# granne/granne

Measured on AMD Instinct MI355X. Metric: queries/sec (recall@10 alongside), 10M x 100-d angular, batch=1024, higher is better.
Workload: dtype f32; 1 GPU; C2 (BASELINE.json configs[1]): 10000000 x 100-d f32 angular, i.i.d. uniform components, batch=1024, ef_search=50, k=10; n_elements=10000000, dim=100, batch=1024, ef_search=50, k=10

## Files before the change

### granne_amd/_lib.py

```python
import ctypes as C
import os

from . import build as _build

F32, I8 = 0, 1
UNUSED = 0xFFFFFFFF
BUILD_ALL = 0xFFFFFFFFFFFFFFFF

OK = 0
ERR_INVALID, ERR_HIP, ERR_NO_DEVICE, ERR_OVERFLOW, ERR_IO = -1, -2, -3, -4, -5

OPT_VISITED_SLOTS, OPT_FORCE_SLOW, OPT_SLOW_SLOTS, OPT_SLOW_BLOCKS, OPT_OVERFLOW_SLOTS = 1, 2, 3, 4, 5
OPT_VISITED16, OPT_VISITED16_LG, OPT_LAST_WALKER, OPT_SEARCH_DEPTH, OPT_INLINE_TAILS, OPT_SEEN_MIN = 6, 7, 8, 9, 10, 11
OPT_SKETCH = 12
OPT_COALESCE, OPT_COALESCE_MAX, OPT_COALESCE_WAIT_US, OPT_COALESCED_LAUNCHES, OPT_COALESCED_QUERIES = 13, 14, 15, 16, 17
COALESCE_CALL_MAX = 64
COALESCE_MAX = 1024
WALKER_NONE, WALKER_REGISTER, WALKER_REGISTER_WIDE, WALKER_GENERAL, WALKER_EXACT = 0, 1, 2, 3, 4
SEARCH_DEPTH = 3
SEARCH_DEPTH_MAX = 16
SHARDED_OPT_DEPTH, SHARDED_OPT_EXCHANGE = 1, 2
SHARDED_EXCHANGE_PEER, SHARDED_EXCHANGE_RCCL = 0, 1
RW_OPT_SMALL_OPS, RW_OPT_SMALL_LAUNCHES, RW_OPT_SORTED_LAUNCHES = 1, 2, 3
RW_SMALL_OPS = 2048
SE_MATERIALIZED, SE_COMPACT = 0, 1


class GranneHipError(RuntimeError):
    def __init__(self, code, message):
        super().__init__("granne_hip error %d: %s" % (code, message))
        self.code = code


class BuildConfig(C.Structure):
    _fields_ = [
        ("layer_multiplier", C.c_float),
        ("expected_num_elements", C.c_uint64),
        ("num_neighbors", C.c_uint32),
# ... 170 lines not shown
```

### granne_amd/csrc/granne_hip.hip

```cpp
#include <hip/hip_runtime.h>

#include <atomic>
#include <chrono>
#include <cstdarg>
#include <cstdio>
#include <cstdlib>
#include <cstring>
#include <memory>
#include <mutex>
#include <string>
#include <type_traits>
#include <vector>

#include "../../include/granne_hip.h"
#include "search_kernel.h"
#include "walk_fast.h"
#include "slow_kernel.h"
#include "util_kernels.h"
#include "brute_force.h"
#include "combiner.h"

using namespace granne_hip;

static_assert(Combiner::DEPTH <= GRANNE_HIP_SEARCH_DEPTH && Combiner::CALL_MAX == GRANNE_HIP_COALESCE_CALL_MAX &&
// ... 28 lines not shown
        if (hipGetDevice(&prev) != hipSuccess) prev = -1;
        ok = hipSetDevice(dev) == hipSuccess;
    }
    ~DeviceGuard() {
        if (prev >= 0) (void)hipSetDevice(prev);
    }
};

extern "C" const char* granne_hip_last_error(void) { return g_last_error.c_str(); }
extern "C" int granne_hip_abi_version(void) { return GRANNE_HIP_ABI_VERSION; }
extern "C" int granne_hip_device_count(int* out_count) {
    if (!out_count) return fail(GRANNE_HIP_ERR_INVALID, "out_count is null");
    int n = 0;
    hipError_t e = hipGetDeviceCount(&n);
    if (e != hipSuccess) {
        *out_count = 0;
        return fail(GRANNE_HIP_ERR_NO_DEVICE, "hipGetDeviceCount: %s", hipGetErrorString(e));
    }
    *out_count = n;
    return GRANNE_HIP_OK;
}

struct EnvKnobs {
    int visited = 0, touch_max = -1, inline_tails = 1, seen_min = -1, bf_b16 = 1, bf_ring = 1, sketch = 1;
    EnvKnobs() {
        auto geti = [](const char* name, int dflt) {
            const char* e = getenv(name);
            return e ? atoi(e) : dflt;
        };
        visited = geti("GRANNE_HIP_VISITED", 0);
        inline_tails = geti("GRANNE_HIP_INLINE_TAILS", 1);
        bf_ring = geti("GRANNE_HIP_BF_RING", 1);
        bf_b16 = geti("GRANNE_HIP_BF_B16", 1);
        seen_min = geti("GRANNE_HIP_SEEN_MIN", -1);
        touch_max = geti("GRANNE_HIP_TOUCH_MAX", -1);
        sketch = geti("GRANNE_HIP_SKETCH", 1);
    }
};
static const EnvKnobs& knobs() {
    static const EnvKnobs k;
    return k;
}

struct ScratchCache {
    struct Block {
        hipStream_t stream;
        uint8_t* p;
        size_t cap;
        uint64_t last_use;
        uint32_t small_runs;
        std::chrono::steady_clock::time_point last_time;
    };
    std::mutex mu;
    std::vector<Block> blocks;
    uint64_t uses = 0;
    std::vector<uint8_t*> graveyard;
    void free_all() {
        for (auto& b : blocks)
            if (b.p) (void)hipFree(b.p);
        blocks.clear();
        for (auto* p : graveyard) (void)hipFree(p);
        graveyard.clear();
    }
};

struct SeDev {
    int device = 0;
    uint32_t dim = 0, tstride = 0;
    uint64_t n_embeddings = 0, n = 0, n_terms = 0;
    float* d_table = nullptr;
    uint64_t* d_offsets = nullptr;
    uint32_t* d_terms = nullptr;
    uint64_t bytes() const { return n_embeddings * tstride * 4u + (n + 1) * 8u + n_terms * 4u; }
    ~SeDev() {
        DeviceGuard g(device);
        if (d_table) (void)hipFree(d_table);
        if (d_offsets) (void)hipFree(d_offsets);
        if (d_terms) (void)hipFree(d_terms);
    }
// ... 16 lines not shown
struct granne_hip_index {
    int device = 0;
    uint32_t dim = 0;
    int dtype = 0;
    uint64_t n_elements = 0;
    uint32_t row_bytes = 0;
    uint32_t row_stride = 0;
    uint8_t* d_elements = nullptr;
    std::shared_ptr<SeDev> se;
    std::vector<LayerHost> layers;
    LayerDev* d_layers = nullptr;
    uint64_t hbm_bytes = 0;
    uint32_t max_dev_width = 32;
    uint64_t opt_visited_slots = 0;
    uint64_t opt_force_slow = 0;
    uint64_t opt_slow_slots = 1u << 18;
    uint64_t opt_slow_blocks = 16;
    uint64_t opt_overflow_slots = 0;
    uint64_t opt_visited16 = 0;
    uint64_t opt_visited16_lg = 0;
    uint64_t opt_inline_tails = 1;
    uint64_t opt_seen_min = 2048;
    uint64_t opt_sketch = 1;
    std::atomic<uint64_t> last_slow_count{0};
    std::atomic<uint64_t> last_walker{0};
    std::mutex norm_mu;
    float* d_inv_norm = nullptr;
    uint8_t* d_sketch = nullptr;
    struct HostCall {
        hipStream_t stream = nullptr;
        uint8_t* d_buf = nullptr;
        size_t d_cap = 0;
        uint8_t* h_pin = nullptr;
        size_t h_cap = 0;
    };
    std::mutex call_mu;
    std::vector<HostCall*> call_free;
    uint64_t opt_coalesce = 0;
    Combiner combiner;
    HostCall* group_call[Combiner::DEPTH] = {};
    ScratchCache scratch;
    struct Flight {
        hipStream_t stream = nullptr;
        hipEvent_t ready = nullptr, done = nullptr;
        bool busy = false;
        uint64_t seq = 0;
// ... 497 lines not shown
        if (value < 1 || value > GRANNE_HIP_SEARCH_DEPTH_MAX) return fail(GRANNE_HIP_ERR_INVALID, "search depth must be in [1, %d]", GRANNE_HIP_SEARCH_DEPTH_MAX);
        std::lock_guard<std::mutex> lk(ix->flight_mu);
        for (auto& f : ix->flights)
            if (f.busy) return fail(GRANNE_HIP_ERR_INVALID, "the depth cannot change while a batch is in flight");
        ix->depth = (uint32_t)value;
        ix->next_flight = 0;
        return GRANNE_HIP_OK;
    }
    case GRANNE_HIP_OPT_INLINE_TAILS: {
        if (value > 1) return fail(GRANNE_HIP_ERR_INVALID, "the inline-tails option is 0 or 1");
        DeviceGuard g(ix->device);
        if (!g.ok) return fail(GRANNE_HIP_ERR_NO_DEVICE, "cannot select HIP device %d", ix->device);
        HIP_TRY(hipDeviceSynchronize());
        ix->opt_inline_tails = value;
        return finish_layers(ix, nullptr);
    }
    case GRANNE_HIP_OPT_SEEN_MIN:
        ix->opt_seen_min = value > 0xFFFFFFFFull ? 0xFFFFFFFFull : value;
        return GRANNE_HIP_OK;
    case GRANNE_HIP_OPT_SKETCH:
        if (value > 1) return fail(GRANNE_HIP_ERR_INVALID, "the sketch option is 0 or 1");
        ix->opt_sketch = value;
        return GRANNE_HIP_OK;
    case GRANNE_HIP_OPT_VISITED16_LG:
        if (value > 12) return fail(GRANNE_HIP_ERR_INVALID, "value out of range");
        ix->opt_visited16_lg = value;
        return GRANNE_HIP_OK;
    case GRANNE_HIP_OPT_COALESCE:
        if (value > 1) return fail(GRANNE_HIP_ERR_INVALID, "the coalesce option is 0 or 1");
        ix->opt_coalesce = value;
        return GRANNE_HIP_OK;
    case GRANNE_HIP_OPT_COALESCE_MAX:
        if (value < 1 || value > GRANNE_HIP_COALESCE_MAX) return fail(GRANNE_HIP_ERR_INVALID, "the coalesce cap must be in [1, %d]", GRANNE_HIP_COALESCE_MAX);
        ix->combiner.set_cap((uint32_t)value);
        return GRANNE_HIP_OK;
    case GRANNE_HIP_OPT_COALESCE_WAIT_US:
        ix->combiner.set_wait_us(value);
        return GRANNE_HIP_OK;
    case GRANNE_HIP_OPT_COALESCED_LAUNCHES:
    case GRANNE_HIP_OPT_COALESCED_QUERIES:
        return fail(GRANNE_HIP_ERR_INVALID, "option %d is read-only", option);
    default:
        return fail(GRANNE_HIP_ERR_INVALID, "unknown option %d", option);
    }
}

extern "C" int granne_hip_index_get_option(const granne_hip_index* ix, int option, uint64_t* value) {
    if (!ix || !value) return fail(GRANNE_HIP_ERR_INVALID, "null argument");
    switch (option) {
    case GRANNE_HIP_OPT_VISITED_SLOTS: *value = ix->opt_visited_slots; return GRANNE_HIP_OK;
    case GRANNE_HIP_OPT_FORCE_SLOW: *value = ix->opt_force_slow; return GRANNE_HIP_OK;
    case GRANNE_HIP_OPT_SLOW_SLOTS: *value = ix->opt_slow_slots; return GRANNE_HIP_OK;
    case GRANNE_HIP_OPT_SLOW_BLOCKS: *value = ix->opt_slow_blocks; return GRANNE_HIP_OK;
    case GRANNE_HIP_OPT_OVERFLOW_SLOTS: *value = ix->opt_overflow_slots; return GRANNE_HIP_OK;
    case GRANNE_HIP_OPT_VISITED16: *value = ix->opt_visited16; return GRANNE_HIP_OK;
    case GRANNE_HIP_OPT_VISITED16_LG: *value = ix->opt_visited16_lg; return GRANNE_HIP_OK;
    case GRANNE_HIP_OPT_LAST_WALKER: *value = ix->last_walker.load(); return GRANNE_HIP_OK;
    case GRANNE_HIP_OPT_SEARCH_DEPTH: *value = ix->depth; return GRANNE_HIP_OK;
    case GRANNE_HIP_OPT_INLINE_TAILS: *value = (!ix->layers.empty() && ix->layers.back().d_adjx) ? 1 : 0; return GRANNE_HIP_OK;
    case GRANNE_HIP_OPT_SEEN_MIN: *value = ix->opt_seen_min; return GRANNE_HIP_OK;
    case GRANNE_HIP_OPT_SKETCH: *value = (ix->opt_sketch && ix->d_sketch && knobs().sketch) ? 1 : 0; return GRANNE_HIP_OK;
    case GRANNE_HIP_OPT_COALESCE: *value = ix->opt_coalesce; return GRANNE_HIP_OK;
    case GRANNE_HIP_OPT_COALESCE_MAX: *value = ix->combiner.cap(); return GRANNE_HIP_OK;
    case GRANNE_HIP_OPT_COALESCE_WAIT_US: *value = ix->combiner.wait_us(); return GRANNE_HIP_OK;
    case GRANNE_HIP_OPT_COALESCED_LAUNCHES: *value = ix->combiner.launches(); return GRANNE_HIP_OK;
    case GRANNE_HIP_OPT_COALESCED_QUERIES: *value = ix->combiner.queries(); return GRANNE_HIP_OK;
    default: return fail(GRANNE_HIP_ERR_INVALID, "unknown option %d", option);
    }
}

extern "C" uint64_t granne_hip_index_last_slow_count(const granne_hip_index* ix) {
    return ix ? ix->last_slow_count.load() : 0;
}

constexpr size_t SLOW_SCRATCH_BUDGET = (size_t)1 << 30;
constexpr uint32_t SCRATCH_MAX_REGIONS = 16384;
constexpr size_t SCRATCH_STATE_OFF = CTL_WORDS * 4;
constexpr size_t SCRATCH_FIXED = SCRATCH_STATE_OFF + (size_t)SCRATCH_MAX_REGIONS * 4;

constexpr size_t SCRATCH_CACHE_STREAMS = 64;
constexpr int SCRATCH_IDLE_SECONDS = 10;
constexpr size_t SCRATCH_SHRINK_ABOVE = 256u << 20;

static int scratch_for(ScratchCache* cache, hipStream_t s, size_t total, uint8_t** out, bool* transient) {
    *transient = false;
    ScratchCache::Block* b = nullptr;
    cache->uses += 1;
    for (auto& x : cache->blocks)
        if (x.stream == s) b = &x;
// ... 35 lines not shown
        HIP_TRY(hipMalloc((void**)&b->p, want));
        b->cap = want;
        HIP_TRY(hipMemsetAsync(b->p, 0, SCRATCH_FIXED, s));
    }
    *out = b->p;
    return GRANNE_HIP_OK;
}

namespace {
struct SearchTarget {
    int device;
    const uint8_t* d_elements;
    uint64_t n_elements;
    uint32_t dim;
    int dtype;
    uint32_t row_bytes, row_stride;
    const LayerDev* d_layers;
    uint32_t n_layers;
    uint32_t max_dev_width;
    uint64_t opt_visited_slots = 0, opt_force_slow = 0, opt_slow_slots = 1u << 18, opt_slow_blocks = 16, opt_overflow_slots = 0;
    uint64_t opt_visited16 = 0;
    uint64_t opt_seen_min = 0xFFFFFFFFull;
    const uint8_t* d_sketch = nullptr;
    const SeDev* se = nullptr;
    ScratchCache* scratch;
    std::atomic<uint64_t>* last_walker = nullptr;

    template <class G>
    SearchTarget(const G* g, const LayerDev* layers, uint32_t n_layers)
        : device(g->device), d_elements(g->d_elements), n_elements(g->n_elements), dim(g->dim), dtype(g->dtype),
          row_bytes(g->row_bytes), row_stride(g->row_stride), d_layers(layers), n_layers(n_layers),
          scratch(&const_cast<G*>(g)->scratch) {
        if constexpr (std::is_same<G, granne_hip_index>::value) {
            max_dev_width = g->max_dev_width;
            opt_visited_slots = g->opt_visited_slots;
            opt_force_slow = g->opt_force_slow;
            opt_slow_slots = g->opt_slow_slots;
            opt_slow_blocks = g->opt_slow_blocks;
            opt_overflow_slots = g->opt_overflow_slots;
            opt_visited16 = g->opt_visited16;
            opt_seen_min = g->opt_seen_min;
            d_sketch = (g->opt_sketch && knobs().sketch) ? g->d_sketch : nullptr;
            last_walker = &const_cast<G*>(g)->last_walker;
            se = g->se.get();
        } else {
            max_dev_width = g->W;
        }
    }
};
}

struct SearchCall {
    const void* queries = nullptr;
    int64_t q_stride = 0;
    uint32_t nq = 0, ef = 0, k = 0;
    uint64_t* ids = nullptr;
    float* dists = nullptr;
    uint32_t* counts = nullptr;
    uint64_t* stats = nullptr;
    uint32_t* status = nullptr;
    hipStream_t stream = nullptr;
    uint32_t* slow_count = nullptr;
    uint32_t* trail = nullptr;
    uint32_t trail_layers = 0;
    hipEvent_t ev_before = nullptr, ev_after = nullptr;
// ... 262 lines not shown
    size_t total = off_sex + (T.se ? (size_t)W.slow_blocks * 64u * T.dim * 4u : 0u);
    struct Bury {
        std::vector<uint8_t*> blocks;
        ~Bury() {
            for (auto* b : blocks) (void)hipFree(b);
        }
    } bury;
    std::unique_lock<std::mutex> cache_lock(T.scratch->mu);
    uint8_t* scratch = nullptr;
    bool transient = false;
    {
        int r = scratch_for(T.scratch, s, total, &scratch, &transient);
        bury.blocks.swap(T.scratch->graveyard);
        if (r) return r;
    }
    struct FreeTransient {
        uint8_t* p;
        hipStream_t s;
        ~FreeTransient() {
            if (p) (void)hipFreeAsync(p, s);
        }
    } free_transient{transient ? scratch : nullptr, s};
    uint32_t* ctl = (uint32_t*)scratch;

    SlowParams sp;
    SearchParams& p = sp.sp;
    p.elements = T.d_elements;
    p.n_elements = T.n_elements;
    p.dim = T.dim;
    p.row_bytes = T.row_bytes;
    p.row_stride = T.row_stride;
    p.layers = T.d_layers;
    p.n_layers = T.n_layers;
    p.queries = (const uint8_t*)c.queries;
    p.q_stride = c.q_stride ? c.q_stride : (int64_t)T.dim * elem_size(T.dtype);
    p.nq = nq;
    p.ef = c.ef;
    p.k = c.k;
    p.out_ids = c.ids;
    p.out_dists = c.dists;
    p.out_counts = c.counts;
    p.out_stats = c.stats;
    p.visited_slots = W.visited_slots;
    p.upper_slots = W.upper_slots;
    p.front_eighths = W.front_eighths;
    p.maxc = W.maxc;
    p.lrow_bytes = W.lrow_bytes;
    p.stage_bytes = W.stage_bytes;
    p.adjspec_bytes = W.adjspec_bytes;
    p.slow_count = ctl + CTL_SLOW_COUNT;
    p.slow_list = (uint32_t*)(scratch + off_list);
    p.force_slow = 0;
    p.spec = 1;
    p.sketch = T.d_sketch;
    p.ovf.tables = (uint32_t*)(scratch + off_ovf);
    p.ovf.state = (uint32_t*)(scratch + SCRATCH_STATE_OFF);
    p.ovf.slots = W.ovf_slots;
    p.ovf.stride = W.ovf_slots;
    p.ovf.regions = W.ovf_regions;
    p.ovf.spilled = c.status ? c.status + 2 : ctl + CTL_SPILLED;
    p.trail_out = c.trail;
    p.trail_layers = c.trail_layers;
    p.n_batches = c.n_batches;
    p.batch_nq = batch_nq;
    for (uint32_t b = 0; b < c.n_batches; ++b) p.batch[b] = c.batches[b];
    sp.ctl = ctl;
    sp.vis = (uint32_t*)(scratch + off_vis);
    sp.pq = (uint64_t*)(scratch + off_pq);
    sp.res = (uint64_t*)(scratch + off_res);
    sp.slots = slots;
    sp.all = W.walker == GRANNE_HIP_WALKER_EXACT ? 1u : 0u;
    sp.status2 = c.status;
    sp.host_status = c.host_status;
    p.se_table = T.se ? T.se->d_table : nullptr;
    p.se_offsets = T.se ? T.se->d_offsets : nullptr;
    p.se_terms = T.se ? T.se->d_terms : nullptr;
    sp.se_x = T.se ? (float*)(scratch + off_sex) : nullptr;
// ... 919 lines not shown
```

### granne_amd/csrc/search_kernel.h

```cpp
#pragma once

#include "dist.h"
#include "wave_prims.h"
#include "sum_embeddings.h"

namespace granne_hip {

constexpr int DT_F32 = 0;
constexpr int DT_I8 = 1;

struct LayerDev {
    const uint32_t* adj;
    uint64_t len;
    uint32_t width;
    uint32_t flags;
    const uint8_t* adjx;
    uint32_t adjx_stride;
    uint32_t reserved;
};
constexpr uint32_t LAYER_TWIN_ROWS = 1u;

constexpr uint32_t SKETCH_LINE = 128u;
constexpr uint32_t SKETCH_META = 112u;
constexpr uint32_t SKETCH_MAX_DIM = 112u;
// ... 17 lines not shown
    const LayerDev* layers;
    uint32_t n_layers;
    const uint8_t* queries;
    int64_t q_stride;
    uint32_t nq;
    uint32_t ef;
    uint32_t k;
    uint64_t* out_ids;
    float* out_dists;
    uint32_t* out_counts;
    uint64_t* out_stats;
    uint32_t visited_slots;
    uint32_t upper_slots;
    uint32_t front_eighths;
    uint32_t maxc;
    uint32_t lrow_bytes;
    uint32_t stage_bytes;
    uint32_t adjspec_bytes;
    uint32_t* slow_count;
    uint32_t* slow_list;
    uint32_t force_slow;
    uint32_t spec;
    const uint8_t* sketch;
    OverflowPool ovf;
    uint32_t* trail_out;
    uint32_t trail_layers;
    uint32_t n_batches;
    uint32_t batch_nq;
    BatchIO batch[MAX_LAUNCH_BATCHES];
    const float* se_table;
    const uint64_t* se_offsets;
    const uint32_t* se_terms;
};
constexpr uint32_t TRAIL_WIDTH = 8;

struct QueryIO {
    const uint8_t* q;
    uint64_t* ids;
    float* dists;
    uint32_t* count;
    uint64_t* stats;
};
__device__ __forceinline__ QueryIO query_io(const SearchParams& p, uint32_t qi) {
    const uint8_t* q = p.queries;
    uint64_t* ids = p.out_ids;
    float* dists = p.out_dists;
// ... 467 lines not shown
```

### granne_amd/csrc/slow_kernel.h

```cpp
#pragma once

#include "search_kernel.h"

namespace granne_hip {

constexpr uint32_t CTL_SLOW_COUNT = 0;
constexpr uint32_t CTL_DONE = 1;
constexpr uint32_t CTL_TAIL_DONE = 2;
constexpr uint32_t CTL_EXHAUSTED = 3;
constexpr uint32_t CTL_LAST_SLOW = 4;
constexpr uint32_t CTL_LAST_EXHAUSTED = 5;
constexpr uint32_t CTL_SPILLED = 6;
constexpr uint32_t CTL_WORDS = 16;

struct SlowParams {
    SearchParams sp;
    uint32_t* ctl;
    uint32_t* vis;
    uint64_t* pq;
    uint64_t* res;
    uint32_t slots;
    uint32_t all;
    uint32_t* status2;
    uint32_t* host_status;
    float* se_x;
};

__device__ inline void gheap_push_min(uint64_t* h, uint32_t& n, uint64_t k) {
    uint32_t i = n++;
    while (i > 0) {
        uint32_t pa = (i - 1) >> 1;
        if (h[pa] <= k) break;
        h[i] = h[pa];
        i = pa;
    }
// ... 252 lines not shown
                uint64_t key = ok ? res[e] : KEY_INF;
                io.ids[e] = ok ? (uint64_t)key_id(key) : ~0ull;
                io.dists[e] = ok ? key_dist(key) : __builtin_inff();
            }
            *io.count = count;
            if (io.stats) {
                io.stats[0] = n_dist;
                io.stats[1] = n_expand;
                io.stats[2] = n_adj;
            }
        }
        __syncthreads();
    }
}

__device__ inline void slow_epilogue(const SlowParams& P, const uint32_t n_blocks, const uint32_t n_slow) {
    __syncthreads();
    if (threadIdx.x == 0) {
        __threadfence();
        if (atomicAdd(P.ctl + CTL_TAIL_DONE, 1u) == n_blocks - 1u) {
            const uint32_t ex = atomicExch(P.ctl + CTL_EXHAUSTED, 0u);
            atomicExch(P.ctl + CTL_LAST_SLOW, n_slow);
            atomicExch(P.ctl + CTL_LAST_EXHAUSTED, ex);
            atomicExch(P.ctl + CTL_SLOW_COUNT, 0u);
            atomicExch(P.ctl + CTL_DONE, 0u);
            atomicExch(P.ctl + CTL_TAIL_DONE, 0u);
        }
    }
}

__device__ __forceinline__ void walker_done(const SlowParams& P) {
    if (threadIdx.x == 0) atomicAdd(P.ctl + CTL_DONE, 1u);
}

template <int DT, bool SE = false>
__device__ inline void tail_block(const SlowParams& P, uint8_t* smem) {
    const uint32_t nq = P.sp.nq;
    const uint32_t me = blockIdx.x - nq, n_blocks = gridDim.x - nq;
    if (threadIdx.x == 0) {
        while (__hip_atomic_load(P.ctl + CTL_DONE, __ATOMIC_RELAXED, __HIP_MEMORY_SCOPE_AGENT) < nq)
            __builtin_amdgcn_s_sleep(24);
    }
    __syncthreads();
    const uint32_t n_slow = __hip_atomic_load(P.ctl + CTL_SLOW_COUNT, __ATOMIC_RELAXED, __HIP_MEMORY_SCOPE_AGENT);
    if (n_slow) slow_walk_list<DT, SE>(P, me, n_blocks, n_slow, smem);
    else if (me == 0 && threadIdx.x == 0 && P.host_status) P.host_status[1] = 0u;
// ... 23 lines not shown
```

### granne_amd/csrc/walk_fast.h

```cpp
#pragma once

#include <type_traits>

#include "slow_kernel.h"

namespace granne_hip {

#ifndef GRANNE_HIP_PHASE_TIMERS
#define GRANNE_HIP_PHASE_TIMERS 0
#endif
#if GRANNE_HIP_PHASE_TIMERS
constexpr uint32_t PHASE_SLOTS = 48, PHASE_QUERIES = 4096;
__device__ uint64_t g_phase[PHASE_QUERIES * PHASE_SLOTS];
#define PT_MARK(i)                                                                   \
    do {                                                                             \
        asm volatile("" ::: "memory");                                               \
        __builtin_amdgcn_sched_barrier(0);                                           \
        const uint64_t now_ = __builtin_amdgcn_s_memtime();                          \
        const uint64_t dt_ = now_ - pt_last;                                         \
        if (pt_bottom) pt_b[i] += dt_; else pt_u[i] += dt_;                          \
        pt_last = now_;                                                              \
        __builtin_amdgcn_sched_barrier(0);                                           \
        asm volatile("" ::: "memory");                                               \
    } while (0)
// ... 799 lines not shown
        asm volatile("" ::: "memory");
#pragma unroll
        for (int s = 0; s < S; ++s) L.key[s] = img[(uint32_t)s * 64u + lane];
        const uint32_t lost = (uint32_t)__builtin_amdgcn_readfirstlane((int)reinterpret_cast<const uint32_t*>(img)[2u * CAP + 1u]);
        theta = (uint32_t)__builtin_amdgcn_readfirstlane((int)reinterpret_cast<const uint32_t*>(img)[2u * (ef - 1u) + 1u]);
        asm volatile("" ::: "memory");
        if (lost == theta && theta != 0xFFFFFFFFu) bail = true;
    }

    __device__ __forceinline__ uint64_t filter_mask(const uint64_t candm, const uint32_t dbits, const uint32_t ef) const {
        uint64_t passm = candm & wave_ballot(dbits <= theta);
        const uint64_t tiem = passm & wave_ballot(dbits == theta);
        if (tiem) {
            const uint32_t w = L.nth_expanded(ef);
            if (w != WPOS_NONE) passm &= ~(tiem & ~wave_ballot(dbits < wkey_hi(L.at(w))));
        }
        return passm;
    }

    __device__ __forceinline__ bool filter(bool cand, float d, uint32_t ef) {
        return __builtin_amdgcn_inverse_ballot_w64(filter_mask(wave_ballot(cand), __float_as_uint(d), ef));
    }

    __device__ __forceinline__ void search_layer_long(const LayerDev& Ly, uint32_t entrypoint, uint32_t ef, uint32_t slots,
                                                      bool d0_known, float d0_value) {
        static_assert(!LONG || (NOVIS && !WIDE && !TOUCH), "lists beyond 1024 keys: no visited set, 32-id layers");
        PT_RESET();
        L.init_list(mslot, lane);
        long_init(0u);
        __syncthreads();
        [[maybe_unused]] const uint8_t* const adjx = XT ? Ly.adjx : nullptr;
        const gptr_u32 adjg = (XT && adjx) ? (gptr_u32)adjx : (gptr_u32)Ly.adj;
        const uint32_t W = (XT && adjx) ? Ly.adjx_stride / 4u : 32u;
        const bool twin_rows = (Ly.flags & LAYER_TWIN_ROWS) != 0u;
        uint32_t pre_id = entrypoint, pre_nb;
        pre_nb = adjg[(size_t)entrypoint * W + R];
        vis.count = 1;
        st.n_dist += 1;
        uint64_t xkey;
        if (d0_known) {
            xkey = wkey(d0_value, entrypoint) | 1ull;
        } else {
            RowRegs r0;
            issue_rows(entrypoint, r0);
            const float d0 = finish_rows(r0);
            xkey = readlane64(wkey(d0, entrypoint), 1) | 1ull;
// ... 331 lines not shown
        for (uint32_t l = 0; l < take; ++l) {
            w.search_layer(p.layers[l], 0u, 1u, p.upper_slots);
            if (w.bail) break;
            const uint32_t found = wkey_id(w.L.at(0));
            if (lane == l) mine = found;
        }
        w.vis.release(p.ovf, lane);
        if (w.bail) {
            hand_over(p, qi);
        } else if (lane < TRAIL_WIDTH) {
            p.trail_out[(size_t)qi * TRAIL_WIDTH + lane] = mine;
        }
        return;
    } else {
        uint32_t entrypoint = 0;
        float ep_dist = 0.0f;
        for (uint32_t l = 0; l < p.n_layers; ++l) {
            const LayerDev Ly = p.layers[l];
            const bool bottom = (l + 1 == p.n_layers);
#if GRANNE_HIP_PHASE_TIMERS
            w.pt_bottom = bottom;
            if (l == 0) w.pt_t0 = __builtin_amdgcn_s_memtime();
#endif
            w.search_layer(Ly, entrypoint, bottom ? p.ef : 1u, bottom ? p.visited_slots : p.upper_slots, l > 0, ep_dist);
            if (w.bail) break;
            if (!bottom) {
                const uint64_t best = w.L.at(0);
                entrypoint = wkey_id(best);
                ep_dist = wkey_dist(best);
            }
        }
        w.vis.release(p.ovf, lane);
        if (w.bail) {
            hand_over(p, qi);
            return;
        }
        uint32_t count;
        const QueryIO io = query_io(p, qi);
        if constexpr (FastWalker<DT, DIM, S, V16, WIDE>::LONG) {
            const uint32_t want = min(p.ef, p.k);
            uint32_t total = 0;
            const uint32_t nm = p.n_layers > 0 ? w.nM : 0u;
            for (uint32_t w0 = 0; w0 < nm && total < want; w0 += 64u) {
                const uint32_t e = w0 + lane;
                const uint64_t v = w.mslot[e < w.CAP ? e : w.CAP - 1u];
                const bool f = e < nm && (((uint32_t)v) & 1u) != 0u;
                const uint64_t em = wave_ballot(f);
// ... 90 lines not shown
```

### granne_amd/index.py

```python
import ctypes as C
import os

import numpy as np

from ._lib import F32, I8, check, lib

DEFAULT_MAX_SEARCH = 200
DEFAULT_NUM_ELEMENTS = 10

_ELEMENT_TYPES = {"angular": (F32, np.float32), "angular_int": (I8, np.int8)}
EMBEDDINGS = "embeddings"


def _p(a):
    return a.ctypes.data_as(C.c_void_p)


def normalize(rows, device=0):
    a = np.array(rows, dtype=np.float32, order="C", copy=True)
    flat = a.reshape(1, -1) if a.ndim == 1 else a
    if flat.size:
        check(lib().granne_hip_normalize_f32(_p(flat), flat.shape[0], flat.shape[1], device))
    return a

# ... 225 lines not shown

    def set_option(self, option, value):
        check(lib().granne_hip_index_set_option(self._h, option, value))

    def get_option(self, option):
        import ctypes as C
        v = C.c_uint64(0)
        check(lib().granne_hip_index_get_option(self._h, option, C.byref(v)))
        return int(v.value)

    def last_slow_count(self):
        return int(lib().granne_hip_index_last_slow_count(self._h))

    @property
    def coalesce(self):
        from ._lib import OPT_COALESCE
        return bool(self.get_option(OPT_COALESCE))

    @coalesce.setter
    def coalesce(self, on):
        from ._lib import OPT_COALESCE
        self.set_option(OPT_COALESCE, 1 if on else 0)

    def _prepare(self, element, prepared):
        if self.element_type == EMBEDDINGS:
            if _is_term_lists(element):
                if getattr(self, "_se", None) is None:
                    raise ValueError("term-id queries need the index's SumEmbeddings container")
                return self._se.create_embeddings(element, normalized=True)
            return np.ascontiguousarray(element, np.float32) if prepared else normalize(element, self.device)
        if prepared:
            return np.ascontiguousarray(element, dtype=self.np_dtype)
        return normalize(element, self.device) if self.element_type == "angular" else quantize(element, self.device)

    def search(self, element, max_search=DEFAULT_MAX_SEARCH, num_elements=DEFAULT_NUM_ELEMENTS, prepared=True):
        terms = self.element_type == EMBEDDINGS and (len(element) == 0 or np.asarray(element).dtype.kind in "iu")
        one = [list(element)] if terms else np.asarray(element).reshape(1, -1)
        ids, dists, counts = self.search_batch(one, max_search, num_elements, prepared)
        return [(int(ids[0, i]), float(dists[0, i])) for i in range(int(counts[0]))]

    def search_batch(self, elements, max_search=DEFAULT_MAX_SEARCH, num_elements=DEFAULT_NUM_ELEMENTS, prepared=True,
                     stats=False):
        q = self._prepare(elements, prepared)
        if q.ndim != 2 or q.shape[1] != self.dim:
            raise ValueError("queries must be [nq, %d]" % self.dim)
        nq, k = q.shape[0], int(num_elements)
# ... 109 lines not shown
```

### include/granne.hpp

```cpp
#pragma once

#include <cmath>
#include <cstdint>
#include <cstring>
#include <memory>
#include <stdexcept>
#include <string>
#include <utility>
#include <vector>

#include "granne_hip.h"

namespace granne {

inline void check(int rc) {
    if (rc != GRANNE_HIP_OK) throw std::runtime_error(std::string("granne_hip: ") + granne_hip_last_error());
}

namespace detail {
struct BuilderDeleter {
    bool armed = true;
    void operator()(granne_hip_builder* b) const { if (armed) granne_hip_builder_destroy(b); }
};
template <class Scalar> struct dtype_of;
// ... 149 lines not shown
        if (keys.size() != len()) throw std::runtime_error("need one key per element");
        std::vector<uint64_t> order(len());
        check(granne_hip_index_reorder_by_keys(h_.get(), keys.data(), order.data()));
        return std::vector<size_t>(order.begin(), order.end());
    }
    void write_index(const std::string& path) const { check(granne_hip_index_save(h_.get(), path.c_str(), nullptr)); }
    void write_elements(const std::string& path) const { check(granne_hip_index_save(h_.get(), nullptr, path.c_str())); }
    std::vector<uint8_t> index_bytes() const {
        void* p = nullptr;
        uint64_t n = 0;
        check(granne_hip_index_encode(h_.get(), &p, &n));
        std::vector<uint8_t> out(static_cast<const uint8_t*>(p), static_cast<const uint8_t*>(p) + n);
        granne_hip_bytes_free(p);
        return out;
    }
    void set_inline_tails(bool keep) { check(granne_hip_index_set_option(h_.get(), GRANNE_HIP_OPT_INLINE_TAILS, keep ? 1 : 0)); }
    void set_seen_min(uint64_t walks) { check(granne_hip_index_set_option(h_.get(), GRANNE_HIP_OPT_SEEN_MIN, walks)); }
    void set_coalesce(bool on) { check(granne_hip_index_set_option(h_.get(), GRANNE_HIP_OPT_COALESCE, on ? 1 : 0)); }
    bool coalesce() const { return get_option(GRANNE_HIP_OPT_COALESCE) != 0; }
    void set_coalesce_max(uint64_t queries) { check(granne_hip_index_set_option(h_.get(), GRANNE_HIP_OPT_COALESCE_MAX, queries)); }
    void set_coalesce_wait_us(uint64_t us) { check(granne_hip_index_set_option(h_.get(), GRANNE_HIP_OPT_COALESCE_WAIT_US, us)); }
    uint64_t coalesced_launches() const { return get_option(GRANNE_HIP_OPT_COALESCED_LAUNCHES); }
    uint64_t coalesced_queries() const { return get_option(GRANNE_HIP_OPT_COALESCED_QUERIES); }
    uint64_t get_option(int option) const {
        uint64_t v = 0;
        check(granne_hip_index_get_option(h_.get(), option, &v));
        return v;
    }
    granne_hip_index* raw() const { return h_.get(); }

private:
    static constexpr int dtype() { return detail::dtype_of<typename decltype(Element::data)::value_type>::value; }
    std::shared_ptr<granne_hip_index> h_;
};

template <class Elements>
class ShardedGranne {
public:
    using Element = typename Elements::Element;
    ShardedGranne(std::vector<Granne<Elements>> shards, const std::vector<uint64_t>& offsets) : shards_(std::move(shards)) {
        if (shards_.empty() || shards_.size() != offsets.size()) throw std::runtime_error("need one offset per shard");
        std::vector<granne_hip_index*> hs;
        for (auto& s : shards_) hs.push_back(s.raw());
        granne_hip_sharded* h = nullptr;
        check(granne_hip_sharded_create(&h, hs.data(), offsets.data(), (uint32_t)hs.size()));
        h_.reset(h, granne_hip_sharded_destroy);
// ... 207 lines not shown
```

### include/granne_hip.h

```cpp
#ifndef GRANNE_HIP_H
#define GRANNE_HIP_H

#include <stddef.h>
#include <stdint.h>

#ifdef __cplusplus
extern "C" {
#endif

#define GRANNE_HIP_ABI_VERSION 3

enum { GRANNE_HIP_F32 = 0, GRANNE_HIP_I8 = 1 };

enum {
    GRANNE_HIP_OK = 0,
    GRANNE_HIP_ERR_INVALID = -1,
    GRANNE_HIP_ERR_HIP = -2,
    GRANNE_HIP_ERR_NO_DEVICE = -3,
    GRANNE_HIP_ERR_OVERFLOW = -4,
    GRANNE_HIP_ERR_IO = -5
};

#define GRANNE_HIP_UNUSED 0xFFFFFFFFu

// ... 280 lines not shown
    GRANNE_HIP_RW_OPT_SORTED_LAUNCHES = 3
};
#define GRANNE_HIP_RW_SMALL_OPS 2048
int granne_hip_rw_builder_set_option(granne_hip_rw_builder* rw, int option, uint64_t value);
int granne_hip_rw_builder_get_option(granne_hip_rw_builder* rw, int option, uint64_t* value);

enum {
    GRANNE_HIP_OPT_VISITED_SLOTS = 1,
    GRANNE_HIP_OPT_FORCE_SLOW = 2,
    GRANNE_HIP_OPT_SLOW_SLOTS = 3,
    GRANNE_HIP_OPT_SLOW_BLOCKS = 4,
    GRANNE_HIP_OPT_OVERFLOW_SLOTS = 5,
    GRANNE_HIP_OPT_VISITED16 = 6,
    GRANNE_HIP_OPT_VISITED16_LG = 7,
    GRANNE_HIP_OPT_LAST_WALKER = 8,
    GRANNE_HIP_OPT_SEARCH_DEPTH = 9,
    GRANNE_HIP_OPT_INLINE_TAILS = 10,
    GRANNE_HIP_OPT_SEEN_MIN = 11,
    GRANNE_HIP_OPT_SKETCH = 12,
    GRANNE_HIP_OPT_COALESCE = 13,
    GRANNE_HIP_OPT_COALESCE_MAX = 14,
    GRANNE_HIP_OPT_COALESCE_WAIT_US = 15,
    GRANNE_HIP_OPT_COALESCED_LAUNCHES = 16,
    GRANNE_HIP_OPT_COALESCED_QUERIES = 17
};
#define GRANNE_HIP_COALESCE_CALL_MAX 64
#define GRANNE_HIP_COALESCE_MAX 1024
enum {
    GRANNE_HIP_WALKER_NONE = 0,
    GRANNE_HIP_WALKER_REGISTER = 1,
    GRANNE_HIP_WALKER_REGISTER_WIDE = 2,
    GRANNE_HIP_WALKER_GENERAL = 3,
    GRANNE_HIP_WALKER_EXACT = 4
};
int granne_hip_index_set_option(granne_hip_index* index, int option, uint64_t value);
int granne_hip_index_get_option(const granne_hip_index* index, int option, uint64_t* value);
uint64_t granne_hip_index_last_slow_count(const granne_hip_index* index);

#ifdef __cplusplus
}
#endif
#endif
```

### rust/granne-hip/src/gpu.rs

```rust
use crate::{angular, angular_int, Index};
use std::marker::PhantomData;
use std::os::raw::{c_char, c_int, c_void};

#[repr(C)] pub struct granne_hip_index { _private: [u8; 0] }
#[repr(C)] pub struct granne_hip_builder { _private: [u8; 0] }
#[repr(C)] pub struct granne_hip_sharded { _private: [u8; 0] }
#[repr(C)] pub struct granne_hip_sum_embeddings { _private: [u8; 0] }
#[repr(C)] pub struct granne_hip_rw_builder { _private: [u8; 0] }

pub const GRANNE_HIP_F32: c_int = 0;
pub const GRANNE_HIP_I8: c_int = 1;
pub const GRANNE_HIP_BUILD_ALL: u64 = u64::MAX;

#[repr(C)]
pub struct granne_hip_build_config {
    pub layer_multiplier: f32,
    pub expected_num_elements: u64,
    pub num_neighbors: u32,
    pub max_search: u32,
    pub reinsert_elements: c_int,
    pub show_progress: c_int,
    pub batch_max: u32,
    pub batch_div: u32,
}
// ... 105 lines not shown
    fn granne_hip_rw_builder_search(rw: *mut granne_hip_rw_builder, query: *const c_void, max_search: u32,
        num_neighbors: u32, out_ids: *mut u64, out_dists: *mut f32, out_count: *mut u32) -> c_int;
    fn granne_hip_rw_builder_len(rw: *mut granne_hip_rw_builder) -> u64;
    fn granne_hip_rw_builder_max_elements(rw: *mut granne_hip_rw_builder) -> u64;
    fn granne_hip_rw_builder_num_layers(rw: *mut granne_hip_rw_builder) -> u32;
    fn granne_hip_rw_builder_layer_len(rw: *mut granne_hip_rw_builder, layer: u32) -> u64;
    fn granne_hip_rw_builder_get_layer(rw: *mut granne_hip_rw_builder, layer: u32, out_rows: *mut u32) -> c_int;
    fn granne_hip_rw_builder_get_element(rw: *mut granne_hip_rw_builder, idx: u64, out: *mut c_void) -> c_int;
    fn granne_hip_rw_builder_save(rw: *mut granne_hip_rw_builder, index_path: *const c_char,
        elements_path: *const c_char) -> c_int;
    fn granne_hip_rw_builder_get_index(rw: *mut granne_hip_rw_builder, out: *mut *mut granne_hip_index) -> c_int;
    fn granne_hip_rw_builder_set_option(rw: *mut granne_hip_rw_builder, option: c_int, value: u64) -> c_int;
    fn granne_hip_rw_builder_get_option(rw: *mut granne_hip_rw_builder, option: c_int, value: *mut u64) -> c_int;
}
pub const GRANNE_HIP_OPT_SEARCH_DEPTH: c_int = 9;
pub const GRANNE_HIP_OPT_INLINE_TAILS: c_int = 10;
pub const GRANNE_HIP_OPT_SEEN_MIN: c_int = 11;
pub const GRANNE_HIP_OPT_SKETCH: c_int = 12;
pub const GRANNE_HIP_OPT_COALESCE: c_int = 13;
pub const GRANNE_HIP_OPT_COALESCE_MAX: c_int = 14;
pub const GRANNE_HIP_OPT_COALESCE_WAIT_US: c_int = 15;
pub const GRANNE_HIP_OPT_COALESCED_LAUNCHES: c_int = 16;
pub const GRANNE_HIP_OPT_COALESCED_QUERIES: c_int = 17;
pub const GRANNE_HIP_RW_OPT_SMALL_OPS: c_int = 1;
pub const GRANNE_HIP_SHARDED_OPT_DEPTH: c_int = 1;
pub const GRANNE_HIP_SHARDED_OPT_EXCHANGE: c_int = 2;
pub const GRANNE_HIP_SHARDED_EXCHANGE_PEER: u64 = 0;
pub const GRANNE_HIP_SHARDED_EXCHANGE_RCCL: u64 = 1;

extern "C" {
    fn granne_hip_abi_version() -> c_int;
    fn granne_hip_index_dtype(index: *const granne_hip_index) -> c_int;
    fn granne_hip_index_device(index: *const granne_hip_index) -> c_int;
    fn granne_hip_index_hbm_bytes(index: *const granne_hip_index) -> u64;
    fn granne_hip_index_last_slow_count(index: *const granne_hip_index) -> u64;
    fn granne_hip_index_set_option(index: *mut granne_hip_index, option: c_int, value: u64) -> c_int;
    fn granne_hip_index_get_option(index: *const granne_hip_index, option: c_int, value: *mut u64) -> c_int;
    fn granne_hip_builder_num_elements(builder: *const granne_hip_builder) -> u64;
    fn granne_hip_sharded_num_shards(sharded: *const granne_hip_sharded) -> u32;
    fn granne_hip_sharded_search(sharded: *mut granne_hip_sharded, query: *const c_void, max_search: u32,
        num_neighbors: u32, out_ids: *mut u64, out_dists: *mut f32, out_count: *mut u32) -> c_int;
    fn granne_hip_sharded_device(sharded: *const granne_hip_sharded) -> c_int;
    fn granne_hip_sharded_shard(sharded: *const granne_hip_sharded, shard: u32) -> *mut granne_hip_index;
    fn granne_hip_sharded_shard_offset(sharded: *const granne_hip_sharded, shard: u32) -> u64;
    fn granne_hip_sharded_get_option(sharded: *const granne_hip_sharded, option: c_int, value: *mut u64) -> c_int;
    fn granne_hip_normalize_f32(rows: *mut f32, n: u64, dim: u32, device_id: c_int) -> c_int;
// ... 222 lines not shown
    }
    pub fn set_search_depth(&mut self, depth: u64) -> std::io::Result<()> {
        check(unsafe { granne_hip_index_set_option(self.handle, GRANNE_HIP_OPT_SEARCH_DEPTH, depth) })
    }
    pub fn set_inline_tails(&mut self, keep: bool) -> std::io::Result<()> {
        check(unsafe { granne_hip_index_set_option(self.handle, GRANNE_HIP_OPT_INLINE_TAILS, keep as u64) })
    }
    pub fn set_seen_min(&mut self, walks: u64) -> std::io::Result<()> {
        check(unsafe { granne_hip_index_set_option(self.handle, GRANNE_HIP_OPT_SEEN_MIN, walks) })
    }
    pub fn set_coalesce(&mut self, on: bool) -> std::io::Result<()> {
        check(unsafe { granne_hip_index_set_option(self.handle, GRANNE_HIP_OPT_COALESCE, on as u64) })
    }
    pub fn set_coalesce_limits(&mut self, max_queries: u64, wait_us: u64) -> std::io::Result<()> {
        check(unsafe { granne_hip_index_set_option(self.handle, GRANNE_HIP_OPT_COALESCE_MAX, max_queries) })?;
        check(unsafe { granne_hip_index_set_option(self.handle, GRANNE_HIP_OPT_COALESCE_WAIT_US, wait_us) })
    }
    pub fn coalesced(&self) -> std::io::Result<(u64, u64)> {
        let (mut launches, mut queries) = (0u64, 0u64);
        check(unsafe { granne_hip_index_get_option(self.handle, GRANNE_HIP_OPT_COALESCED_LAUNCHES, &mut launches) })?;
        check(unsafe { granne_hip_index_get_option(self.handle, GRANNE_HIP_OPT_COALESCED_QUERIES, &mut queries) })?;
        Ok((launches, queries))
    }
    pub fn len(&self) -> usize { unsafe { granne_hip_index_len(self.handle) as usize } }
    pub fn num_layers(&self) -> usize { unsafe { granne_hip_index_num_layers(self.handle) as usize } }
    pub fn layer_len(&self, layer: usize) -> usize { unsafe { granne_hip_index_layer_len(self.handle, layer as u32) as usize } }
    pub fn get_neighbors(&self, index: usize, layer: usize) -> Vec<usize> {
        let mut buf = vec![0u32; 512];
        let mut n = 0u32;
        check(unsafe { granne_hip_index_get_neighbors(self.handle, index as u64, layer as u32, buf.as_mut_ptr(),
            buf.len() as u32, &mut n) }).expect("granne_hip_index_get_neighbors");
        buf[..n as usize].iter().map(|&i| i as usize).collect()
    }
    pub fn reorder(&mut self, _show_progress: bool) -> Vec<usize> {
        let mut order = vec![0u64; self.len()];
        check(unsafe { granne_hip_index_reorder(self.handle, order.as_mut_ptr()) }).expect("granne_hip_index_reorder");
        order.into_iter().map(|i| i as usize).collect()
    }
    pub fn reorder_by_keys(&mut self, keys: &[u64], _show_progress: bool) -> Vec<usize> {
        assert_eq!(self.len(), keys.len());
        let mut order = vec![0u64; self.len()];
        check(unsafe { granne_hip_index_reorder_by_keys(self.handle, keys.as_ptr(), order.as_mut_ptr()) })
            .expect("granne_hip_index_reorder_by_keys");
        order.into_iter().map(|i| i as usize).collect()
    }
    pub fn dists(&self, element: &E::Vector, indices: &[usize]) -> Vec<f32> {
// ... 316 lines not shown
```

Before: 13.84 million queries/s.

## Add greedy single-candidate descent path for ef=1 upper layers

Adds a specialised greedy walk for upper HNSW layers where ef is 1. It keeps only the current best node in a register and uses wave-wide min reductions instead of the general candidate-list search_layer machinery. On ties or NaNs it falls back to the regular search and counts the fallbacks in a scratch control word, which is exposed through a new read-only option. It is enabled by default for f32 non-wide register walkers. The added code paths raise register pressure, and a fallback repeats the walk.

```diff
diff --git a/granne_amd/_lib.py b/granne_amd/_lib.py
--- a/granne_amd/_lib.py
+++ b/granne_amd/_lib.py
@@ -14,6 +14,7 @@
 OPT_VISITED16, OPT_VISITED16_LG, OPT_LAST_WALKER, OPT_SEARCH_DEPTH, OPT_INLINE_TAILS, OPT_SEEN_MIN = 6, 7, 8, 9, 10, 11
 OPT_SKETCH = 12
 OPT_COALESCE, OPT_COALESCE_MAX, OPT_COALESCE_WAIT_US, OPT_COALESCED_LAUNCHES, OPT_COALESCED_QUERIES = 13, 14, 15, 16, 17
+OPT_UPPER_DESCENT, OPT_DESCENT_FALLBACKS = 18, 19
 COALESCE_CALL_MAX = 64
 COALESCE_MAX = 1024
 WALKER_NONE, WALKER_REGISTER, WALKER_REGISTER_WIDE, WALKER_GENERAL, WALKER_EXACT = 0, 1, 2, 3, 4
diff --git a/granne_amd/csrc/granne_hip.hip b/granne_amd/csrc/granne_hip.hip
--- a/granne_amd/csrc/granne_hip.hip
+++ b/granne_amd/csrc/granne_hip.hip
@@ -74,7 +74,7 @@
 }
 
 struct EnvKnobs {
-    int visited = 0, touch_max = -1, inline_tails = 1, seen_min = -1, bf_b16 = 1, bf_ring = 1, sketch = 1;
+    int visited = 0, touch_max = -1, inline_tails = 1, seen_min = -1, bf_b16 = 1, bf_ring = 1, sketch = 1, upper_descent = 1;
     EnvKnobs() {
         auto geti = [](const char* name, int dflt) {
             const char* e = getenv(name);
@@ -86,6 +86,7 @@
         bf_b16 = geti("GRANNE_HIP_BF_B16", 1);
         seen_min = geti("GRANNE_HIP_SEEN_MIN", -1);
         touch_max = geti("GRANNE_HIP_TOUCH_MAX", -1);
+        upper_descent = geti("GRANNE_HIP_UPPER_DESCENT", 1);
         sketch = geti("GRANNE_HIP_SKETCH", 1);
     }
 };
@@ -107,6 +108,7 @@
     std::vector<Block> blocks;
     uint64_t uses = 0;
     std::vector<uint8_t*> graveyard;
+    uint8_t* last = nullptr;
     void free_all() {
         for (auto& b : blocks)
             if (b.p) (void)hipFree(b.p);
@@ -169,6 +171,7 @@
     uint64_t opt_inline_tails = 1;
     uint64_t opt_seen_min = 2048;
     uint64_t opt_sketch = 1;
+    uint64_t opt_upper_descent = 1;
     std::atomic<uint64_t> last_slow_count{0};
     std::atomic<uint64_t> last_walker{0};
     std::mutex norm_mu;
@@ -712,6 +715,10 @@
         if (value > 1) return fail(GRANNE_HIP_ERR_INVALID, "the sketch option is 0 or 1");
         ix->opt_sketch = value;
         return GRANNE_HIP_OK;
+    case GRANNE_HIP_OPT_UPPER_DESCENT:
+        if (value > 1) return fail(GRANNE_HIP_ERR_INVALID, "the upper-descent option is 0 or 1");
+        ix->opt_upper_descent = value;
+        return GRANNE_HIP_OK;
     case GRANNE_HIP_OPT_VISITED16_LG:
         if (value > 12) return fail(GRANNE_HIP_ERR_INVALID, "value out of range");
         ix->opt_visited16_lg = value;
@@ -729,6 +736,7 @@
         return GRANNE_HIP_OK;
     case GRANNE_HIP_OPT_COALESCED_LAUNCHES:
     case GRANNE_HIP_OPT_COALESCED_QUERIES:
+    case GRANNE_HIP_OPT_DESCENT_FALLBACKS:
         return fail(GRANNE_HIP_ERR_INVALID, "option %d is read-only", option);
     default:
         return fail(GRANNE_HIP_ERR_INVALID, "unknown option %d", option);
@@ -755,6 +763,19 @@
     case GRANNE_HIP_OPT_COALESCE_WAIT_US: *value = ix->combiner.wait_us(); return GRANNE_HIP_OK;
     case GRANNE_HIP_OPT_COALESCED_LAUNCHES: *value = ix->combiner.launches(); return GRANNE_HIP_OK;
     case GRANNE_HIP_OPT_COALESCED_QUERIES: *value = ix->combiner.queries(); return GRANNE_HIP_OK;
+    case GRANNE_HIP_OPT_UPPER_DESCENT: *value = (ix->opt_upper_descent && knobs().upper_descent) ? 1 : 0; return GRANNE_HIP_OK;
+    case GRANNE_HIP_OPT_DESCENT_FALLBACKS: {
+        DeviceGuard g(ix->device);
+        if (!g.ok) return fail(GRANNE_HIP_ERR_NO_DEVICE, "cannot select HIP device %d", ix->device);
+        HIP_TRY(hipDeviceSynchronize());
+        ScratchCache& sc = const_cast<granne_hip_index*>(ix)->scratch;
+        std::lock_guard<std::mutex> lk(sc.mu);
+        uint32_t v = 0;
+        for (auto& b : sc.blocks)
+            if (b.p && b.p == sc.last) HIP_TRY(hipMemcpy(&v, b.p + CTL_LAST_DESCENT_FALLBACK * 4, 4, hipMemcpyDeviceToHost));
+        *value = v;
+        return GRANNE_HIP_OK;
+    }
     default: return fail(GRANNE_HIP_ERR_INVALID, "unknown option %d", option);
     }
 }
@@ -836,6 +857,7 @@
     uint64_t opt_visited16 = 0;
     uint64_t opt_seen_min = 0xFFFFFFFFull;
     const uint8_t* d_sketch = nullptr;
+    uint32_t upper_descent = knobs().upper_descent ? 1u : 0u;
     const SeDev* se = nullptr;
     ScratchCache* scratch;
     std::atomic<uint64_t>* last_walker = nullptr;
@@ -855,6 +877,7 @@
             opt_visited16 = g->opt_visited16;
             opt_seen_min = g->opt_seen_min;
             d_sketch = (g->opt_sketch && knobs().sketch) ? g->d_sketch : nullptr;
+            upper_descent = (g->opt_upper_descent && knobs().upper_descent) ? 1u : 0u;
             last_walker = &const_cast<G*>(g)->last_walker;
             se = g->se.get();
         } else {
@@ -1163,6 +1186,7 @@
         }
     } free_transient{transient ? scratch : nullptr, s};
     uint32_t* ctl = (uint32_t*)scratch;
+    T.scratch->last = transient ? nullptr : scratch;
 
     SlowParams sp;
     SearchParams& p = sp.sp;
@@ -1194,6 +1218,8 @@
     p.force_slow = 0;
     p.spec = 1;
     p.sketch = T.d_sketch;
+    p.upper_descent = T.upper_descent;
+    p.descent_fallbacks = ctl + CTL_DESCENT_FALLBACK;
     p.ovf.tables = (uint32_t*)(scratch + off_ovf);
     p.ovf.state = (uint32_t*)(scratch + SCRATCH_STATE_OFF);
     p.ovf.slots = W.ovf_slots;
diff --git a/granne_amd/csrc/search_kernel.h b/granne_amd/csrc/search_kernel.h
--- a/granne_amd/csrc/search_kernel.h
+++ b/granne_amd/csrc/search_kernel.h
@@ -63,6 +63,8 @@
     uint32_t force_slow;
     uint32_t spec;
     const uint8_t* sketch;
+    uint32_t upper_descent;
+    uint32_t* descent_fallbacks;
     OverflowPool ovf;
     uint32_t* trail_out;
     uint32_t trail_layers;
diff --git a/granne_amd/csrc/slow_kernel.h b/granne_amd/csrc/slow_kernel.h
--- a/granne_amd/csrc/slow_kernel.h
+++ b/granne_amd/csrc/slow_kernel.h
@@ -11,6 +11,8 @@
 constexpr uint32_t CTL_LAST_SLOW = 4;
 constexpr uint32_t CTL_LAST_EXHAUSTED = 5;
 constexpr uint32_t CTL_SPILLED = 6;
+constexpr uint32_t CTL_DESCENT_FALLBACK = 7;
+constexpr uint32_t CTL_LAST_DESCENT_FALLBACK = 8;
 constexpr uint32_t CTL_WORDS = 16;
 
 struct SlowParams {
@@ -309,6 +311,7 @@
             const uint32_t ex = atomicExch(P.ctl + CTL_EXHAUSTED, 0u);
             atomicExch(P.ctl + CTL_LAST_SLOW, n_slow);
             atomicExch(P.ctl + CTL_LAST_EXHAUSTED, ex);
+            atomicExch(P.ctl + CTL_LAST_DESCENT_FALLBACK, atomicExch(P.ctl + CTL_DESCENT_FALLBACK, 0u));
             atomicExch(P.ctl + CTL_SLOW_COUNT, 0u);
             atomicExch(P.ctl + CTL_DONE, 0u);
             atomicExch(P.ctl + CTL_TAIL_DONE, 0u);
diff --git a/granne_amd/csrc/walk_fast.h b/granne_amd/csrc/walk_fast.h
--- a/granne_amd/csrc/walk_fast.h
+++ b/granne_amd/csrc/walk_fast.h
@@ -845,6 +845,125 @@
         return __builtin_amdgcn_inverse_ballot_w64(filter_mask(wave_ballot(cand), __float_as_uint(d), ef));
     }
 
+    static constexpr bool DESCENT = F32 && !GEN && NOVIS && !WIDE && !LONG_LIST && S <= 2;
+
+    __device__ __forceinline__ static uint32_t wave_min_u32(uint32_t v) {
+        v = min(v, (uint32_t)__builtin_amdgcn_update_dpp((int)v, (int)v, 0x111 , 0xf, 0xf, false));
+        v = min(v, (uint32_t)__builtin_amdgcn_update_dpp((int)v, (int)v, 0x112 , 0xf, 0xf, false));
+        v = min(v, (uint32_t)__builtin_amdgcn_update_dpp((int)v, (int)v, 0x114 , 0xf, 0xf, false));
+        v = min(v, (uint32_t)__builtin_amdgcn_update_dpp((int)v, (int)v, 0x118 , 0xf, 0xf, false));
+        return min(min(readlane32(v, 15), readlane32(v, 31)), min(readlane32(v, 47), readlane32(v, 63)));
+    }
+
+    __device__ __forceinline__ bool descend_layer(const LayerDev& Ly, uint32_t entrypoint, bool d0_known, float d0_value, uint64_t& out) {
+        static_assert(DESCENT, "unrolled f32 rows, 32-id layers, no visited set, lists in registers");
+        PT_RESET();
+        const WalkStats st0 = st;
+        [[maybe_unused]] const uint8_t* const adjx = XT ? Ly.adjx : nullptr;
+        const gptr_u32 adjg = (XT && adjx) ? (gptr_u32)adjx : (gptr_u32)Ly.adj;
+        const uint32_t W = (XT && adjx) ? Ly.adjx_stride / 4u : 32u;
+        uint32_t next_nb = adjg[(size_t)entrypoint * W + R];
+        st.n_dist += 1;
+        uint32_t xbits;
+        if (d0_known) {
+            xbits = __float_as_uint(d0_value);
+        } else {
+            RowRegs r0;
+            issue_rows(entrypoint, r0);
+            const float d0 = finish_rows(r0);
+            xbits = readlane32(__float_as_uint(d0), 1);
+        }
+        if constexpr (SEEN) vcache_reset(entrypoint);
+        uint32_t xid = entrypoint;
+        bool tied = false, nan = __uint_as_float(xbits) != __uint_as_float(xbits);
+        RowRegs rr;
+        PT_WAIT_VM();
+        PT_MARK(7);
+        while (!nan) {
+            st.n_expand += 1;
+            uint32_t nb;
+            asm volatile("v_mov_b32 %0, %1" : "=v"(nb) : "v"(next_nb));
+            PT_MARK(0);
+            PT_WAIT_VM();
+            PT_MARK(8);
+            PT_COUNT();
+            const uint64_t unused = wave_ballot(nb == ID_EMPTY);
+            const uint32_t nvalid = unused ? ((uint32_t)__builtin_ctzll(unused) >> 1) : 32u;
+            st.n_adj += nvalid;
+            theta = xbits;
+            [[maybe_unused]] uint64_t seenm = 0, skipm = 0;
+            if constexpr (SEEN) {
+                const bool seen = vcache[vcache_slot(nb)] == nb;
+                seenm = wave_ballot(seen);
+                bool go = !seen && nb != ID_EMPTY;
+                if constexpr (SK) {
+                    if (p.sketch && sk_on && theta < 0x7F800000u) {
+                        skipm = sketch_rejects(nb, go, rr);
+                        go = go && ((skipm >> lane) & 1ull) == 0ull;
+                    }
+                }
+                if (go) {
+                    const uint8_t* tails = nullptr;
+                    if constexpr (XT) {
+                        if (adjx) tails = adjx + (size_t)xid * Ly.adjx_stride + 128u + R * XTAILB;
+                    }
+                    issue_rows(nb, rr, tails);
+                }
+                if (nb != ID_EMPTY && !__builtin_amdgcn_inverse_ballot_w64(seenm)) vcache[vcache_slot(nb)] = nb;
+            } else {
+                uint32_t fill = readlane32(nb, 0);
+                asm("" : "+v"(fill));
+                fill = fill != ID_EMPTY ? fill : xid;
+                const uint8_t* tails = nullptr;
+                if constexpr (XT) {
+                    if (adjx) tails = adjx + (size_t)xid * Ly.adjx_stride + 128u + (nb != ID_EMPTY ? R : 0u) * XTAILB;
+                }
+                issue_rows(nb != ID_EMPTY ? nb : fill, rr, tails);
+            }
+            asm volatile("" ::: "memory");
+            __builtin_amdgcn_sched_barrier(0);
+            PT_MARK(1);
+            const uint64_t fm = 0x5555555555555555ull & ~unused & ~seenm;
+            PT_WAIT_VM();
+            PT_MARK(3);
+            const float d = finish_rows(rr);
+            st.n_dist += (uint32_t)__popcll(fm);
+            PT_PIN(d);
+            PT_MARK(4);
+            const uint32_t dbits = __float_as_uint(d);
+            const uint64_t candm = (fm << 1) & ~skipm;
+            if (candm & wave_ballot(d != d)) {
+                nan = true;
+                break;
+            }
+            const uint64_t passm = candm & wave_ballot(dbits < xbits);
+            if (passm == 0) break;
+            const bool pass = __builtin_amdgcn_inverse_ballot_w64(passm);
+            const uint32_t minb = wave_min_u32(pass ? dbits : 0xFFFFFFFFu);
+            uint64_t winm = passm & wave_ballot(dbits == minb);
+            tied = false;
+            if (winm & (winm - 1)) {
+                const bool in = __builtin_amdgcn_inverse_ballot_w64(winm);
+                const uint32_t wid = wave_min_u32(in ? nb : 0xFFFFFFFFu);
+                const uint64_t same = wave_ballot(nb == wid);
+                tied = (winm & ~same) != 0;
+                winm &= same;
+            }
+            xid = readlane32(nb, (uint32_t)__builtin_ctzll(winm));
+            xbits = minb;
+            uint32_t xv = xid;
+            asm("" : "+v"(xv));
+            next_nb = adjg[(size_t)xv * W + R];
+            PT_MARK(5);
+        }
+        if (tied || nan) {
+            st = st0;
+            return false;
+        }
+        out = (((uint64_t)xbits << 32) | ((uint64_t)xid << 1)) | 1ull;
+        return true;
+    }
+
     __device__ __forceinline__ void search_layer_long(const LayerDev& Ly, uint32_t entrypoint, uint32_t ef, uint32_t slots,
                                                       bool d0_known, float d0_value) {
         static_assert(!LONG || (NOVIS && !WIDE && !TOUCH), "lists beyond 1024 keys: no visited set, 32-id layers");
@@ -1222,7 +1341,26 @@
             w.pt_bottom = bottom;
             if (l == 0) w.pt_t0 = __builtin_amdgcn_s_memtime();
 #endif
-            w.search_layer(Ly, entrypoint, bottom ? p.ef : 1u, bottom ? p.visited_slots : p.upper_slots, l > 0, ep_dist);
+            const uint32_t ef_l = bottom ? p.ef : 1u;
+            bool descended = false;
+            if constexpr (FastWalker<DT, DIM, S, V16, WIDE>::DESCENT) {
+                if (p.upper_descent && ef_l == 1u) {
+                    uint64_t best;
+                    descended = w.descend_layer(Ly, entrypoint, l > 0, ep_dist, best);
+                    if (descended) {
+                        entrypoint = wkey_id(best);
+                        ep_dist = wkey_dist(best);
+                        if (bottom) {
+                            w.L.init_list(w.mslot, lane);
+                            w.L.set_first(best, lane);
+                        }
+                    } else if (lane == 0) {
+                        atomicAdd(p.descent_fallbacks, 1u);
+                    }
+                }
+            }
+            if (descended) continue;
+            w.search_layer(Ly, entrypoint, ef_l, bottom ? p.visited_slots : p.upper_slots, l > 0, ep_dist);
             if (w.bail) break;
             if (!bottom) {
                 const uint64_t best = w.L.at(0);
diff --git a/granne_amd/index.py b/granne_amd/index.py
--- a/granne_amd/index.py
+++ b/granne_amd/index.py
@@ -271,6 +271,20 @@
         from ._lib import OPT_COALESCE
         self.set_option(OPT_COALESCE, 1 if on else 0)
 
+    @property
+    def upper_descent(self):
+        from ._lib import OPT_UPPER_DESCENT
+        return bool(self.get_option(OPT_UPPER_DESCENT))
+
+    @upper_descent.setter
+    def upper_descent(self, on):
+        from ._lib import OPT_UPPER_DESCENT
+        self.set_option(OPT_UPPER_DESCENT, 1 if on else 0)
+
+    def descent_fallbacks(self):
+        from ._lib import OPT_DESCENT_FALLBACKS
+        return self.get_option(OPT_DESCENT_FALLBACKS)
+
     def _prepare(self, element, prepared):
         if self.element_type == EMBEDDINGS:
             if _is_term_lists(element):
diff --git a/include/granne.hpp b/include/granne.hpp
--- a/include/granne.hpp
+++ b/include/granne.hpp
@@ -195,6 +195,8 @@
     void set_coalesce_wait_us(uint64_t us) { check(granne_hip_index_set_option(h_.get(), GRANNE_HIP_OPT_COALESCE_WAIT_US, us)); }
     uint64_t coalesced_launches() const { return get_option(GRANNE_HIP_OPT_COALESCED_LAUNCHES); }
     uint64_t coalesced_queries() const { return get_option(GRANNE_HIP_OPT_COALESCED_QUERIES); }
+    void set_upper_descent(bool on) { check(granne_hip_index_set_option(h_.get(), GRANNE_HIP_OPT_UPPER_DESCENT, on ? 1 : 0)); }
+    uint64_t descent_fallbacks() const { return get_option(GRANNE_HIP_OPT_DESCENT_FALLBACKS); }
     uint64_t get_option(int option) const {
         uint64_t v = 0;
         check(granne_hip_index_get_option(h_.get(), option, &v));
diff --git a/include/granne_hip.h b/include/granne_hip.h
--- a/include/granne_hip.h
+++ b/include/granne_hip.h
@@ -326,7 +326,9 @@
     GRANNE_HIP_OPT_COALESCE_MAX = 14,
     GRANNE_HIP_OPT_COALESCE_WAIT_US = 15,
     GRANNE_HIP_OPT_COALESCED_LAUNCHES = 16,
-    GRANNE_HIP_OPT_COALESCED_QUERIES = 17
+    GRANNE_HIP_OPT_COALESCED_QUERIES = 17,
+    GRANNE_HIP_OPT_UPPER_DESCENT = 18,
+    GRANNE_HIP_OPT_DESCENT_FALLBACKS = 19
 };
 #define GRANNE_HIP_COALESCE_CALL_MAX 64
 #define GRANNE_HIP_COALESCE_MAX 1024
diff --git a/rust/granne-hip/src/gpu.rs b/rust/granne-hip/src/gpu.rs
--- a/rust/granne-hip/src/gpu.rs
+++ b/rust/granne-hip/src/gpu.rs
@@ -151,6 +151,8 @@
 pub const GRANNE_HIP_OPT_COALESCE_WAIT_US: c_int = 15;
 pub const GRANNE_HIP_OPT_COALESCED_LAUNCHES: c_int = 16;
 pub const GRANNE_HIP_OPT_COALESCED_QUERIES: c_int = 17;
+pub const GRANNE_HIP_OPT_UPPER_DESCENT: c_int = 18;
+pub const GRANNE_HIP_OPT_DESCENT_FALLBACKS: c_int = 19;
 pub const GRANNE_HIP_RW_OPT_SMALL_OPS: c_int = 1;
 pub const GRANNE_HIP_SHARDED_OPT_DEPTH: c_int = 1;
 pub const GRANNE_HIP_SHARDED_OPT_EXCHANGE: c_int = 2;
@@ -419,6 +421,14 @@
         check(unsafe { granne_hip_index_get_option(self.handle, GRANNE_HIP_OPT_COALESCED_QUERIES, &mut queries) })?;
         Ok((launches, queries))
     }
+    pub fn set_upper_descent(&mut self, on: bool) -> std::io::Result<()> {
+        check(unsafe { granne_hip_index_set_option(self.handle, GRANNE_HIP_OPT_UPPER_DESCENT, on as u64) })
+    }
+    pub fn descent_fallbacks(&self) -> std::io::Result<u64> {
+        let mut v = 0u64;
+        check(unsafe { granne_hip_index_get_option(self.handle, GRANNE_HIP_OPT_DESCENT_FALLBACKS, &mut v) })?;
+        Ok(v)
+    }
     pub fn len(&self) -> usize { unsafe { granne_hip_index_len(self.handle) as usize } }
     pub fn num_layers(&self) -> usize { unsafe { granne_hip_index_num_layers(self.handle) as usize } }
     pub fn layer_len(&self, layer: usize) -> usize { unsafe { granne_hip_index_layer_len(self.handle, layer as u32) as usize } }
```

Result: no change. 13.86 million queries/s, median of 3 (+0.1%).
